# Tariq-Abuhashim/semantic-slam

Measured on AMD Instinct MI355X. Metric: Mvoxels/sec integrated, 512³ grid @ 640×480 depth; achieved HBM GB/s %peak, higher is better.
Workload: dtype f32

## Files before the change

include/tsdf_hip_diag.h:

```cpp
#ifndef TSDF_HIP_DIAG_H
#define TSDF_HIP_DIAG_H

#include "tsdf_hip.h"

#ifdef __cplusplus
extern "C" {
#endif


int tsdf_integrate_sequence_timed(tsdf_volume *vol, const float *depth_dev, const float *cam2world,
                                  int32_t n_frames, float *elapsed_ms);

int tsdf_integrate_frames_timed(tsdf_volume *vol, const float *const *depth_dev, const uint8_t *const *masks_dev,
                                const float *cam2world, int32_t n_frames, float *elapsed_ms);


int tsdf_probe_graph_replay(tsdf_volume *vol, const float *depth_dev, const float *cam2world, int32_t n_frames,
                            int32_t iters, float *ms_launches, float *ms_graph);

int tsdf_probe_stream(tsdf_volume *vol, int32_t non_temporal, int32_t n_iters, float *elapsed_ms);


int tsdf_selftest_fastdiv(int32_t device, uint64_t seed, uint64_t n_samples, float fx, float cx,
                          uint64_t *mismatches, float first_bad[4]);

int tsdf_selftest_fastdiv_band(int32_t device, uint64_t seed, uint64_t n_samples, uint64_t *mismatches,
                               float first_bad[4]);

int tsdf_selftest_round(int32_t device, uint64_t *mismatches, float first_bad[4]);

int tsdf_selftest_tile_tables(int32_t device, const float *depth_dev, const uint8_t *mask_dev, int32_t im_height,
                              int32_t im_width, float max_depth, uint64_t *mismatches);


int32_t tsdf_frames_per_launch(const tsdf_volume *vol);
int tsdf_shortcut_stats(tsdf_volume *vol, int32_t enable, uint64_t counts_out[3]);
int tsdf_brick_list_stats(tsdf_volume *vol, uint64_t counts_out[4]);
int tsdf_classification_info(tsdf_volume *vol, double info_out[2]);

int tsdf_summary_stats(tsdf_volume *vol, uint64_t out[3]);
int tsdf_summary_words(tsdf_volume *vol, uint32_t *out_host, int64_t capacity, int64_t *count);

int tsdf_store_stats(tsdf_volume *vol, int64_t out[9]);

int tsdf_last_cam2base(const tsdf_volume *vol, float out[16]);


int tsdf_set_kernel_variant(tsdf_volume *vol, int32_t variant);

int tsdf_set_brick_shape(tsdf_volume *vol, int32_t quads, int32_t rows, int32_t slices);
int tsdf_brick_shape(const tsdf_volume *vol, int32_t shape_out[3]);
int tsdf_default_brick_shape(const tsdf_config *cfg, int32_t shape_out[3]);

#ifdef __cplusplus
}
#endif
#endif
```

semantic_slam_amd/capi.py:

```python
import ctypes as C
import os

import numpy as np

_PKG = os.path.dirname(os.path.abspath(__file__))
LIB_PATH = os.environ.get("TSDF_HIP_LIB") or os.path.join(_PKG, "libtsdf_hip.so")

ABI_SYMBOLS = [
    "tsdf_config_default", "tsdf_create", "tsdf_destroy", "tsdf_reset", "tsdf_integrate",
    "tsdf_integrate_u16", "tsdf_convert_depth_u16", "tsdf_set_deferral",
    "tsdf_integrate_device", "tsdf_integrate_cam2base", "tsdf_integrate_masked_device",
    "tsdf_integrate_frames_device",
    "tsdf_sync", "tsdf_download", "tsdf_copy_slices", "tsdf_upload", "tsdf_refresh_summary", "tsdf_device_ptrs", "tsdf_slab_voxels", "tsdf_frames_per_launch", "tsdf_shortcut_stats", "tsdf_brick_list_stats", "tsdf_classification_info", "tsdf_store_stats", "tsdf_summary_stats", "tsdf_summary_words",
    "tsdf_get_config", "tsdf_last_cam2base", "tsdf_set_stream", "tsdf_get_stream",
    "tsdf_count_surface", "tsdf_extract_surface", "tsdf_extract_crossings", "tsdf_extract_mesh", "tsdf_save_mesh_ply", "tsdf_save_mesh_welded_ply", "tsdf_save_ply", "tsdf_save_bin", "tsdf_load_bin", "tsdf_save_state", "tsdf_load_state",
    "tsdf_integrate_sequence_timed", "tsdf_integrate_frames_timed", "tsdf_probe_graph_replay", "tsdf_probe_stream", "tsdf_selftest_fastdiv", "tsdf_selftest_fastdiv_band", "tsdf_selftest_round", "tsdf_selftest_tile_tables", "tsdf_set_kernel_variant", "tsdf_set_brick_shape", "tsdf_brick_shape", "tsdf_default_brick_shape", "tsdf_last_error",
    "tsdf_version", "tsdf_multiply_matrix", "tsdf_invert_matrix",
    "tsdf_labels_enable", "tsdf_compose_labels", "tsdf_integrate_labels_device", "tsdf_integrate_frames_labels_device",
    "tsdf_download_labels",
    "tsdf_colour_enable", "tsdf_integrate_colour_device", "tsdf_integrate_rgbd", "tsdf_download_colour",
    "tsdf_raycast_params_default", "tsdf_raycast_device", "tsdf_raycast", "tsdf_batch_raycast_device",
    "tsdf_track_params_default", "tsdf_track", "tsdf_track_system",
    "tsdf_batch_track", "tsdf_batch_track_system", "tsdf_track_member_systems",
    "tsdf_fuse_params_default", "tsdf_fuse_volume",
    "tsdf_align_params_default", "tsdf_fuse_pose_default", "tsdf_align_volume", "tsdf_align_system", "tsdf_fuse_volume_at",
    "tsdf_extent_params_default", "tsdf_volume_extent", "tsdf_batch_extents", "tsdf_group_extent", "tsdf_extent_combine",
    "tsdf_extent_metric", "tsdf_extent_regrid",
    "tsdf_associate_params_default", "tsdf_associate_count", "tsdf_associate_assign", "tsdf_batch_associate",
    "tsdf_segment_params_default", "tsdf_segmenter_create", "tsdf_segmenter_destroy", "tsdf_segmenter_set_stream",
    "tsdf_segment_depth_device", "tsdf_segment_refine_masks_device", "tsdf_segment_frame",
    "tsdf_object_origin", "tsdf_batch_create", "tsdf_batch_destroy", "tsdf_batch_size", "tsdf_batch_volume",
    "tsdf_batch_integrate_device", "tsdf_batch_sync",
    "tsdf_group_create", "tsdf_group_destroy", "tsdf_group_size", "tsdf_group_voxels", "tsdf_group_volume",
    "tsdf_group_integrate", "tsdf_group_integrate_frames", "tsdf_group_set_deferral", "tsdf_group_sync", "tsdf_group_reset", "tsdf_group_download",
    "tsdf_group_extract_surface", "tsdf_group_extract_crossings", "tsdf_group_extract_mesh",
    "tsdf_group_save_ply", "tsdf_group_save_mesh_ply", "tsdf_group_save_bin",
]
DIAG_SYMBOLS = [
    "tsdf_integrate_sequence_timed", "tsdf_integrate_frames_timed",
    "tsdf_probe_graph_replay", "tsdf_probe_stream",
    "tsdf_selftest_fastdiv", "tsdf_selftest_fastdiv_band", "tsdf_selftest_round", "tsdf_selftest_tile_tables",
    "tsdf_shortcut_stats", "tsdf_brick_list_stats", "tsdf_classification_info", "tsdf_store_stats", "tsdf_summary_stats", "tsdf_summary_words", "tsdf_frames_per_launch", "tsdf_last_cam2base",
    "tsdf_set_kernel_variant", "tsdf_set_brick_shape", "tsdf_brick_shape", "tsdf_default_brick_shape",
]


class TsdfError(RuntimeError):
    pass


SHIPPED_VARIANTS = (0, 1, 3, 7, 8)


def experiments_build():
    return b"+experiments" in load().tsdf_version()


def variants(*wanted):
    exp = experiments_build()
    return [v for v in wanted if v in SHIPPED_VARIANTS or exp]


class TsdfConfig(C.Structure):
    _fields_ = [
        ("im_height", C.c_int32), ("im_width", C.c_int32),
# ... 116 lines not shown
    L.tsdf_destroy.argtypes = [vp]
    L.tsdf_reset.argtypes = [vp]
    L.tsdf_integrate.argtypes = [vp, vp, vp]
    L.tsdf_set_deferral.argtypes = [vp, C.c_int32]
    L.tsdf_integrate_u16.argtypes = [vp, vp, C.c_float, C.c_int32, C.c_int32, vp]
    L.tsdf_convert_depth_u16.argtypes = [vp, vp, vp, C.c_float, C.c_int32, C.c_int32]
    L.tsdf_integrate_device.argtypes = [vp, vp, vp]
    L.tsdf_integrate_cam2base.argtypes = [vp, vp, vp]
    L.tsdf_integrate_masked_device.argtypes = [vp, vp, vp, vp]
    L.tsdf_integrate_frames_device.argtypes = [vp, vp, vp, vp, C.c_int32]
    L.tsdf_sync.argtypes = [vp]
    L.tsdf_download.argtypes = [vp, vp, vp]
    L.tsdf_upload.argtypes = [vp, vp, vp]
    L.tsdf_copy_slices.argtypes = [vp, C.c_int32, C.c_int32, vp, vp]
    L.tsdf_refresh_summary.argtypes = [vp]
    L.tsdf_device_ptrs.argtypes = [vp, C.POINTER(vp), C.POINTER(vp)]
    L.tsdf_slab_voxels.argtypes = [vp]
    L.tsdf_slab_voxels.restype = C.c_int64
    L.tsdf_frames_per_launch.argtypes = [vp]
    L.tsdf_frames_per_launch.restype = C.c_int32
    L.tsdf_shortcut_stats.argtypes = [vp, C.c_int32, vp]
    L.tsdf_classification_info.argtypes = [vp, vp]
    L.tsdf_brick_list_stats.argtypes = [vp, vp]
    if hasattr(L, "tsdf_store_stats"):
        L.tsdf_store_stats.argtypes = [vp, i64p]
    if hasattr(L, "tsdf_summary_stats"):
        L.tsdf_summary_stats.argtypes = [vp, vp]
    if hasattr(L, "tsdf_summary_words"):
        L.tsdf_summary_words.argtypes = [vp, vp, C.c_int64, i64p]
    L.tsdf_get_config.argtypes = [vp, C.POINTER(TsdfConfig)]
    L.tsdf_last_cam2base.argtypes = [vp, vp]
    L.tsdf_set_stream.argtypes = [vp, vp]
    L.tsdf_get_stream.argtypes = [vp, C.POINTER(vp)]
    L.tsdf_count_surface.argtypes = [vp, C.c_float, i64p]
    L.tsdf_extract_surface.argtypes = [vp, C.c_float, vp, C.c_int64, i64p]
    L.tsdf_extract_crossings.argtypes = [vp, vp, vp, C.c_float, vp, C.c_int64, i64p]
    L.tsdf_extract_mesh.argtypes = [vp, vp, vp, C.c_float, vp, C.c_int64, i64p]
    L.tsdf_save_mesh_ply.argtypes = [vp, C.c_char_p, C.c_float]
    L.tsdf_save_mesh_welded_ply.argtypes = [vp, C.c_char_p, C.c_float]
    L.tsdf_save_ply.argtypes = [vp, C.c_char_p, C.c_float]
    L.tsdf_save_bin.argtypes = [vp, C.c_char_p]
    L.tsdf_load_bin.argtypes = [vp, C.c_char_p]
    L.tsdf_save_state.argtypes = [vp, C.c_char_p]
    L.tsdf_load_state.argtypes = [vp, C.c_char_p]
    L.tsdf_integrate_sequence_timed.argtypes = [vp, vp, vp, C.c_int32, f32p]
    L.tsdf_integrate_frames_timed.argtypes = [vp, vp, vp, vp, C.c_int32, f32p]
# ... 133 lines not shown


def invert_matrix(m):
    out = np.zeros(16, np.float32)
    m = _f32(m, 16)
    ok = load().tsdf_invert_matrix(m.ctypes.data, out.ctypes.data)
    return bool(ok), out


def selftest_fastdiv(n_samples, seed=1, device=0, fx=535.4, cx=320.1):
    cnt = C.c_uint64()
    bad = (C.c_float * 4)()
    check(load().tsdf_selftest_fastdiv(device, seed, n_samples, fx, cx, C.byref(cnt), bad), "tsdf_selftest_fastdiv")
    return cnt.value, list(bad)


def selftest_fastdiv_band(n_samples, seed=1, device=0):
    cnt = C.c_uint64()
    bad = (C.c_float * 4)()
    check(load().tsdf_selftest_fastdiv_band(device, seed, n_samples, C.byref(cnt), bad), "tsdf_selftest_fastdiv_band")
    return cnt.value, list(bad)


def object_origin(depth_ptr, mask_ptr, h, w, K, device=0):
    k = _f32(K, 9)
    out = np.empty(3, np.float32)
    check(load().tsdf_object_origin(device, depth_ptr, mask_ptr, h, w, k.ctypes.data, out.ctypes.data), "tsdf_object_origin")
    return out


def raycast_params_default(cfg):
    p = RaycastParams()
    check(load().tsdf_raycast_params_default(C.byref(cfg), C.byref(p)), "tsdf_raycast_params_default")
    return p


def track_params_default(cfg):
    p = TrackParams()
    check(load().tsdf_track_params_default(C.byref(cfg), C.byref(p)), "tsdf_track_params_default")
    return p


def fuse_params_default(cfg):
    p = FuseParams()
    check(load().tsdf_fuse_params_default(C.byref(cfg), C.byref(p)), "tsdf_fuse_params_default")
    return p
# ... 184 lines not shown
        return self

    def __exit__(self, *exc):
        self.close()

    def __del__(self):
        try:
            self.close()
        except Exception:
            pass

    @property
    def n_voxels(self):
        return int(self.lib.tsdf_slab_voxels(self._h))

    def shortcut_stats(self, enable=True):
        out = (C.c_uint64 * 3)()
        check(self.lib.tsdf_shortcut_stats(self._h, 1 if enable else 0, out), "tsdf_shortcut_stats")
        return tuple(int(x) for x in out)

    def brick_list_stats(self):
        out = (C.c_uint64 * 4)()
        check(self.lib.tsdf_brick_list_stats(self._h, out), "tsdf_brick_list_stats")
        return tuple(int(x) for x in out)

    def classification_info(self):
        out = (C.c_double * 2)()
        check(self.lib.tsdf_classification_info(self._h, out), "tsdf_classification_info")
        return float(out[0]), int(out[1])

    def store_stats(self):
        out = (C.c_int64 * 9)()
        check(self.lib.tsdf_store_stats(self._h, out), "tsdf_store_stats")
        return {name: tuple(int(x) for x in out[3 * k:3 * k + 3]) for k, name in enumerate(("frames", "masks", "tables"))}

    def summary_stats(self):
        out = (C.c_uint64 * 3)()
        check(self.lib.tsdf_summary_stats(self._h, out), "tsdf_summary_stats")
        return tuple(int(x) for x in out)

    def summary_words(self):
        n = C.c_int64(0)
        check(self.lib.tsdf_summary_words(self._h, None, 0, C.byref(n)), "tsdf_summary_words")
        out = np.zeros(int(n.value), np.uint32)
        if out.size:
            check(self.lib.tsdf_summary_words(self._h, out.ctypes.data, out.size, C.byref(n)), "tsdf_summary_words")
# ... 540 lines not shown
```

semantic_slam_amd/csrc/host_derive.h:

```cpp
#pragma once
#include <algorithm>
#include <cmath>
#include <cstddef>
#include <cstdint>

#include "tsdf_hip.h"

namespace tsdf_host {

inline bool brick_shape_ok(const tsdf_config &c, int q, int r, int s)
{
    return c.dim_x % 4 == 0 && q >= 1 && r >= 1 && s >= 1 && q * r * s <= 64 && (c.dim_x / 4) % q == 0 &&
           (long long)s * c.dim_x * c.dim_y < (1ll << 30);
}

inline void choose_brick_default(const tsdf_config &c, int &bq, int &br, int &bs)
{
    bq = 0; br = 0; bs = 1;
    if (c.dim_x % 4 != 0) return;
    const int quads = c.dim_x / 4;
    const int nz = c.z_end - c.z_begin;
    double best = 1e300;
    for (int q = 1; q <= 64 && q <= quads; ++q) {
        if (quads % q) continue;
// ... 176 lines not shown
constexpr uint32_t kSummaryOnes = 1u, kSummarySane = 2u, kSummaryRun = 4u;
constexpr int kRunCountShift = 8;
constexpr uint32_t kMaxRunCount = (1u << 24) - 1;
constexpr uint32_t kSummaryFresh = kSummaryOnes | kSummarySane | kSummaryRun;

TSDF_HOST_DEVICE inline bool word_has_run(uint32_t word) { return (word & kSummaryRun) != 0u; }
TSDF_HOST_DEVICE inline uint32_t word_run_count(uint32_t word) { return word >> kRunCountShift; }
TSDF_HOST_DEVICE inline uint32_t word_with_run(uint32_t low, uint32_t c)
{
    return (low & (kSummaryOnes | kSummarySane)) | kSummaryRun | (c << kRunCountShift);
}
TSDF_HOST_DEVICE inline uint32_t word_without_run(uint32_t word) { return word & (kSummaryOnes | kSummarySane); }

TSDF_HOST_DEVICE inline uint32_t word_after_update(uint32_t word, bool touched, bool all_updated, bool left_not_one)
{
    if (!touched) return word;
    if (left_not_one) word &= ~kSummaryOnes;
    if (!word_has_run(word)) return word;
    const uint32_t c = word_run_count(word);
    if (!all_updated || c >= kMaxRunCount) return word_without_run(word);
    return word_with_run(word, c + 1u);
}

struct Regions {
    size_t add(size_t bytes) { const size_t at = (end_ + 255) / 256 * 256; end_ = at + bytes; return at; }
    size_t total() const { return end_; }
    size_t end_ = 0;
};

}
```

semantic_slam_amd/csrc/tsdf_diag.hip.h:

```cpp
#pragma once

namespace {

template <typename Queue>
int time_on_stream(tsdf_volume *v, const char *who, float *elapsed_ms, Queue &&queue)
{
    Event e0, e1;
    HIP_TRY(event_create(e0, hipEventDefault));
    HIP_TRY(event_create(e1, hipEventDefault));
    HIP_TRY(hipEventRecord(e0, v->stream));
    const int rc = queue();
    hipError_t er = hipEventRecord(e1, v->stream);
    hipError_t es = hipEventSynchronize(e1);
    float ms = 0.f;
    hipError_t et = hipEventElapsedTime(&ms, e0, e1);
    if (rc) return rc;
    if (er != hipSuccess || es != hipSuccess || et != hipSuccess)
        return fail(TSDF_ERR_HIP, "%s: event timing failed", who);
    *elapsed_ms = ms;
    return TSDF_OK;
}

int frames_timed(tsdf_volume *v, const float *const *depth_dev, const uint8_t *const *masks_dev,
                 const float *cam2world, int32_t n_frames, float *elapsed_ms, const char *who)
// ... 108 lines not shown
    if (e == hipSuccess) e = hipMemcpy(first_bad, d_bad, 4 * sizeof(float), hipMemcpyDeviceToHost);
    if (e != hipSuccess) return fail(TSDF_ERR_HIP, "tsdf_selftest_fastdiv: %s", hipGetErrorString(e));
    *mismatches = cnt;
    return TSDF_OK;
}

int tsdf_selftest_fastdiv_band(int32_t device, uint64_t seed, uint64_t n_samples, uint64_t *mismatches, float first_bad[4])
{
    if (!mismatches || !first_bad) return fail(TSDF_ERR_INVALID, "tsdf_selftest_fastdiv_band: NULL argument");
    HIP_TRY(hipSetDevice(device));
    DevPtr<unsigned long long> d_cnt;
    DevPtr<float> d_bad;
    HIP_TRY(dev_alloc(d_cnt, sizeof(unsigned long long)));
    HIP_TRY(dev_alloc(d_bad, 4 * sizeof(float)));
    HIP_TRY(hipMemset(d_cnt, 0, sizeof(unsigned long long)));
    HIP_TRY(hipMemset(d_bad, 0, 4 * sizeof(float)));
    hipLaunchKernelGGL(tsdfk::selftest_fastdiv_band, dim3(256 * 8), dim3(256), 0, 0, seed, n_samples, d_cnt, d_bad);
    hipError_t e = hipGetLastError();
    if (e == hipSuccess) e = hipDeviceSynchronize();
    unsigned long long cnt = 0;
    if (e == hipSuccess) e = hipMemcpy(&cnt, d_cnt, sizeof cnt, hipMemcpyDeviceToHost);
    if (e == hipSuccess) e = hipMemcpy(first_bad, d_bad, 4 * sizeof(float), hipMemcpyDeviceToHost);
    if (e != hipSuccess) return fail(TSDF_ERR_HIP, "tsdf_selftest_fastdiv_band: %s", hipGetErrorString(e));
    *mismatches = cnt;
    return TSDF_OK;
}

int tsdf_selftest_round(int32_t device, uint64_t *mismatches, float first_bad[4])
{
    if (!mismatches || !first_bad) return fail(TSDF_ERR_INVALID, "tsdf_selftest_round: NULL argument");
    HIP_TRY(hipSetDevice(device));
    DevPtr<unsigned long long> d_cnt;
    DevPtr<float> d_bad;
    HIP_TRY(dev_alloc(d_cnt, sizeof(unsigned long long)));
    HIP_TRY(dev_alloc(d_bad, 4 * sizeof(float)));
    HIP_TRY(hipMemset(d_cnt, 0, sizeof(unsigned long long)));
    HIP_TRY(hipMemset(d_bad, 0, 4 * sizeof(float)));
    hipLaunchKernelGGL(tsdfk::selftest_round, dim3(256 * 8), dim3(256), 0, 0, d_cnt, d_bad);
    hipError_t e = hipGetLastError();
    if (e == hipSuccess) e = hipDeviceSynchronize();
    unsigned long long cnt = 0;
    if (e == hipSuccess) e = hipMemcpy(&cnt, d_cnt, sizeof cnt, hipMemcpyDeviceToHost);
    if (e == hipSuccess) e = hipMemcpy(first_bad, d_bad, 4 * sizeof(float), hipMemcpyDeviceToHost);
    if (e != hipSuccess) return fail(TSDF_ERR_HIP, "tsdf_selftest_round: %s", hipGetErrorString(e));
    *mismatches = cnt;
    return TSDF_OK;
// ... 90 lines not shown
    }
    *mismatches = bad;
    return TSDF_OK;
}


int32_t tsdf_frames_per_launch(const tsdf_volume *v)
{
    if (!v) return 0;
    return can_fuse(v) ? frames_per_launch(v) : 1;
}

int tsdf_shortcut_stats(tsdf_volume *v, int32_t enable, uint64_t counts_out[3])
{
    if (!v) return fail(TSDF_ERR_INVALID, "tsdf_shortcut_stats: NULL handle");
    int rc = bind_device(v);
    if (rc) return rc;
    HIP_TRY(hipStreamSynchronize(v->stream));
    if (counts_out) {
        unsigned int h[3] = {0, 0, 0};
        if (v->d_shortcut_stats) HIP_TRY(hipMemcpy(h, v->d_shortcut_stats, sizeof h, hipMemcpyDeviceToHost));
        for (int i = 0; i < 3; ++i) counts_out[i] = h[i];
    }
    if (enable && !v->d_shortcut_stats) HIP_TRY(dev_alloc(v->d_shortcut_stats, 8 * sizeof(unsigned int)));
    if (v->d_shortcut_stats) {
        if (enable) HIP_TRY(hipMemset(v->d_shortcut_stats, 0, 8 * sizeof(unsigned int)));
        else v->d_shortcut_stats.reset();
    }
    return TSDF_OK;
}

int tsdf_brick_list_stats(tsdf_volume *v, uint64_t counts_out[4])
{
    if (!v || !counts_out) return fail(TSDF_ERR_INVALID, "tsdf_brick_list_stats: NULL argument");
    int rc = bind_device(v);
    if (rc) return rc;
    HIP_TRY(hipStreamSynchronize(v->stream));
    unsigned int h[8] = {0, 0, 0, 0, 0, 0, 0, 0};
    if (v->d_shortcut_stats) HIP_TRY(hipMemcpy(h, v->d_shortcut_stats, sizeof h, hipMemcpyDeviceToHost));
    for (int i = 0; i < 4; ++i) counts_out[i] = h[3 + i];
    return TSDF_OK;
}

int tsdf_classification_info(tsdf_volume *v, double info_out[2])
{
    if (!v || !info_out) return fail(TSDF_ERR_INVALID, "tsdf_classification_info: NULL argument");
    int rc = bind_device(v);
    if (rc) return rc;
    HIP_TRY(hipStreamSynchronize(v->stream));
    if (v->rb_stream) HIP_TRY(hipStreamSynchronize(v->rb_stream));
    if (v->claims_pending && hipEventQuery(v->claims_done) == hipSuccess) {
        v->claim_fraction = claims_read_back(v);
        v->claims_pending = false;
        v->claims_known = true;
    }
    info_out[0] = v->claims_known ? v->claim_fraction : -1.0;
    info_out[1] = (double)v->launches_unclassified;
    return TSDF_OK;
}

int tsdf_summary_stats(tsdf_volume *v, uint64_t out[3])
{
    if (!v || !out) return fail(TSDF_ERR_INVALID, "tsdf_summary_stats: NULL argument");
// ... 85 lines not shown
```

semantic_slam_amd/csrc/tsdf_kernels.hip.h:

```cpp
#pragma once
#include <hip/hip_runtime.h>
#include <stdint.h>
#include <type_traits>

#include "host_derive.h"

namespace tsdfk {

struct IntegrateParams {
    const float *depth;
    const uint8_t *mask;
    float *tsdf;
    float *weight;
    float fx, fy, cx, cy;
    float rx0, rx1, rx2;
    float ry0, ry1, ry2;
    float rz0, rz1, rz2;
    float tx, ty, tz;
    float ox, oy, oz;
    float vs, trunc, max_depth;
    int dim_x, dim_y;
    int nz, z_begin;
    int H, W;
    int xgroups;
    uint32_t *flags;
    int nseg;
    int quads_per_row, quads_per_slice, chunks_per_slice;
    int brick_q, brick_r, brick_s, bricks_per_group, brick_groups;
    int brick_q_magic, brick_per_magic;
    int fast_ok;
// ... 450 lines not shown
        const uint32_t mode = h2 & 7u;
        uint32_t dm = h0 & 0x7fffffu;
        if (mode == 1) dm = 0x7fffffu; else if (mode == 2) dm = 0u; else if (mode == 3) dm &= 0x7u;
        const uint32_t de = 127u - 20u + (h0 >> 23) % 41u;
        const float d = __uint_as_float((de << 23) | dm);
        uint32_t ne = 127u - 81u + (h1 >> 23) % 142u;
        if (mode >= 6) ne = de - 2u + (h1 >> 23) % 5u;
        if (ne > 127u + 60u) ne = 127u + 60u;
        uint32_t nm = h1 & 0x7fffffu;
        if (mode == 4) nm = 0x7fffffu; else if (mode == 5) nm = dm;
        if (ne == 127u + 60u) nm = 0u;
        float n = __uint_as_float((((h2 >> 3) & 1u) << 31) | (ne << 23) | nm);
        if (((h2 >> 5) & 63u) == 0u) n = 0.0f;
        if (((h2 >> 5) & 63u) == 1u) n = __uint_as_float(0x7fc00000u | (h2 >> 12));
        const float q = fast_div_r(n, d, refined_rcp(d));
        const float r = n / d;
        const bool same = __float_as_uint(q) == __float_as_uint(r) || (q != q && r != r);
        if (!same) {
            if (atomicAdd(mismatch, 1ull) == 0ull) { first_bad[0] = n; first_bad[1] = d; first_bad[2] = q; first_bad[3] = r; }
        }
    }
}

__global__ __launch_bounds__(256) void selftest_round(unsigned long long *mismatch, float *first_bad)
{
    const uint64_t stride = (uint64_t)gridDim.x * blockDim.x;
    const uint64_t n_pos = 0x4B800001ull, n_neg = 0x3F000000ull;
    for (uint64_t i = (uint64_t)blockIdx.x * blockDim.x + threadIdx.x; i < n_pos + n_neg; i += stride) {
        const uint32_t bits = i < n_pos ? (uint32_t)i : (0x80000000u + (uint32_t)(i - n_pos));
        const float u = __uint_as_float(bits);
        if (!(u > -0.5f)) continue;
        const int want = (int)roundf(u);
        const int got = round_half_up_i32(u);
        if (got != want) {
            if (atomicAdd(mismatch, 1ull) == 0ull) { first_bad[0] = u; first_bad[1] = (float)got; first_bad[2] = (float)want; first_bad[3] = 0.f; }
        }
    }
}

template <bool NT>
__global__ __launch_bounds__(256) void stream_rmw(float *tsdf, float *weight, size_t n_quads, float one,
                                                  float zero)
{
    const size_t stride = (size_t)gridDim.x * blockDim.x;
    for (size_t q = (size_t)blockIdx.x * blockDim.x + threadIdx.x; q < n_quads; q += stride) {
        float4 t = vol_load<NT>(tsdf + 4 * q);
// ... 112 lines not shown
```

semantic_slam_amd/csrc/tsdf_multiframe.hip.h:

```cpp
#pragma once
#include "launch_geometry.h"
#include "tsdf_kernels.hip.h"

namespace tsdfk {

constexpr int kMaxFramesPerLaunch = 32;
constexpr int kFineTile = 4;
constexpr int kFineLevels = 3;
__host__ __device__ inline size_t fine_table_elems(int fw, int fh) { return (size_t)kFineLevels * kFineLevels * fw * fh; }

struct FramePose {
    const float *depth;
    const uint8_t *mask;
    float rx0, ry0, rx1, ry1, rx2, ry2, rz0, rz1, rz2, tz, tx, ty;
    int fast_ok;
    float cz_margin;
    const uint16_t *label_im;
    const float *score_im;
    const float2 *tiles;
    float cz_short;
    float cz_pad;
};

constexpr int kListBuckets = 64;
// ... 517 lines not shown
    cls[id] = (uint8_t)c;
}

struct LabelState {
    uint16_t *label;
    float *fp, *bp;
    float prob_thd;
};

struct MultiParamsInline {
    IntegrateParams common;
    FramePose frames[kMaxFramesPerLaunch];
    int n_frames;
    LabelState labels;
    int z_fastest;
#ifdef TSDF_EXPERIMENTS
    const unsigned int *super_mask;
    int nz_super;
#endif
};

constexpr int kSuperZ = 4;

template <int R, bool NT, bool FLAT, bool LABELS = false, bool MASKS = true, bool SHORT = false, bool BRICK = false, bool EAGER_W = false>
__device__ __forceinline__ void multi_body(const IntegrateParams &p, const FramePose *__restrict__ frames,
                                           const int n_frames, const int b0, const int b1, const int lz,
                                           const LabelState ls = LabelState(), const unsigned int free_frames = 0u,
                                           const unsigned int skip_frames = 0u)
{
    static_assert(!SHORT || R == 1, "patch classification is written for one row per lane");
    static_assert(!LABELS || R == 1, "label fusion rides on the one-row kernel");
    static_assert(!FLAT || R == 1, "the flat mapping handles one quad per lane");
    static_assert(!BRICK || (R == 1 && !FLAT), "bricks are their own mapping");
    static_assert(!EAGER_W || BRICK, "eager weights are for the bricks of a work list");
    int xg, gy0;
    size_t row0, flag0;
    size_t brick_base = 0;
    unsigned int lane_byte = 0u;
    uint32_t flag32 = 0u;
    constexpr bool kBuf = BRICK && !NT;
    __amdgpu_buffer_rsrc_t t_buf, w_buf;
    auto load_quad = [&](const bool tsdf, const int r) -> float4 {
        if constexpr (kBuf) {
            const v4u v = __builtin_amdgcn_raw_buffer_load_b128(tsdf ? t_buf : w_buf, (int)lane_byte, 0, 0);
            return make_float4(__uint_as_float(v.x), __uint_as_float(v.y), __uint_as_float(v.z), __uint_as_float(v.w));
        } else {
            return vol_load<NT>((tsdf ? p.tsdf : p.weight) + row0 + (size_t)r * p.dim_x);
        }
    };
    auto store_quad = [&](const bool tsdf, const int r, const float4 q) {
        if constexpr (kBuf) {
            const v4u v = {__float_as_uint(q.x), __float_as_uint(q.y), __float_as_uint(q.z), __float_as_uint(q.w)};
            __builtin_amdgcn_raw_buffer_store_b128(v, tsdf ? t_buf : w_buf, (int)lane_byte, 0, 0);
        } else {
            vol_store<NT>((tsdf ? p.tsdf : p.weight) + row0 + (size_t)r * p.dim_x, q);
        }
    };
// ... 49 lines not shown
        t4[r] = make_float4(1.f, 1.f, 1.f, 1.f);
        w4[r] = make_float4(0.f, 0.f, 0.f, 0.f);
        touched[r] = tchanged[r] = false;
    }
    bool have_w = false;
    if constexpr (EAGER_W) {
        w4[0] = load_quad(false, 0);
        have_w = true;
    }

    float bxv[4], byv[R];
#pragma unroll
    for (int j = 0; j < 4; ++j) bxv[j] = p.ox + (float)(xg * 4 + j) * p.vs;
#pragma unroll
    for (int r = 0; r < R; ++r) byv[r] = p.oy + (float)(gy0 + r) * p.vs;
    const float bz = p.oz + (float)gz * p.vs;
    const v2f F = {p.fx, p.fy}, C = {p.cx, p.cy};
    const float trunc_r1 = refined_rcp(p.trunc);
    bool fast_frame = false;

    float diff[R][4];
    bool upd[R][4], rowany[R], bandr[R];
    bool any = false, band = false;
    auto apply_frame = [&]() __attribute__((always_inline)) {
#pragma unroll
        for (int r = 0; r < R; ++r) {
            if (rowany[r] && !touched[r]) {
                if (!have_w) w4[r] = load_quad(false, r);
                if (!(fl[r] & 1u)) t4[r] = load_quad(true, r);
                touched[r] = true;
            }
        }
        float dist[R][4];
        if (__ballot(band) != 0ull) {
            if (fast_frame && p.trunc_fast != 0) {
#pragma unroll
                for (int r = 0; r < R; ++r)
#pragma unroll
                    for (int j = 0; j < 4; ++j) dist[r][j] = fminf(1.0f, fast_div_r(diff[r][j], p.trunc, trunc_r1));
            } else {
#pragma unroll
                for (int r = 0; r < R; ++r)
#pragma unroll
                    for (int j = 0; j < 4; ++j) dist[r][j] = fminf(1.0f, diff[r][j] / p.trunc);
            }
        } else {
#pragma unroll
            for (int r = 0; r < R; ++r)
#pragma unroll
                for (int j = 0; j < 4; ++j) dist[r][j] = 1.0f;
        }

#pragma unroll
        for (int r = 0; r < R; ++r) {
            if (__ballot(!(ones[r] && (fl[r] & 2u)) || bandr[r]) == 0ull) {
                if (upd[r][0]) w4[r].x += 1.0f;
                if (upd[r][1]) w4[r].y += 1.0f;
                if (upd[r][2]) w4[r].z += 1.0f;
                if (upd[r][3]) w4[r].w += 1.0f;
                continue;
            }
            float tv[4] = {t4[r].x, t4[r].y, t4[r].z, t4[r].w};
            float wv[4] = {w4[r].x, w4[r].y, w4[r].z, w4[r].w};
            float num[4], wn[4];
            const bool wave_band = __ballot(bandr[r]) != 0ull;
            bool need = false;
#pragma unroll
            for (int j = 0; j < 4; ++j) {
                wn[j] = wv[j] + 1.0f;
                num[j] = tv[j] * wv[j] + dist[r][j];
            }
            if (!wave_band) {
#pragma unroll
// ... 163 lines not shown
                for (int r = 0; r < R; ++r)
#pragma unroll
                    for (int j = 0; j < 4; ++j) dval[r][j] = dval[r][j] * (mval[r][j] >= 128 ? 1.0f : 0.0f);
            }
        }

#pragma unroll
        for (int r = 0; r < R; ++r) {
            rowany[r] = false;
            bandr[r] = false;
#pragma unroll
            for (int j = 0; j < 4; ++j) {
                const float d = dval[r][j];
                const float df = d - pcz[r][j];
                diff[r][j] = df;
                const bool u = !((d <= 0.0f) | (d > p.max_depth)) & !(df <= -p.trunc);
                upd[r][j] = u;
                rowany[r] |= u;
                bandr[r] |= u & !(df >= p.trunc);
            }
            band |= bandr[r];
            any |= rowany[r];
        }
        if (__ballot(any) == 0ull) continue;

        if constexpr (LABELS) {
            if (q.label_im != nullptr && __ballot(band) != 0ull) {
                uint16_t lab_in[4];
                float sc_in[4];
                bool hit = false;
#pragma unroll
                for (int j = 0; j < 4; ++j) {
                    const bool seen = upd[0][j] & (diff[0][j] < p.trunc);
                    lab_in[j] = 0;
                    sc_in[j] = 0.0f;
                    if (seen) { lab_in[j] = q.label_im[pixel[0][j]]; sc_in[j] = q.score_im[pixel[0][j]]; }
                    hit |= lab_in[j] != 0;
                }
                if (hit) {
                    ushort4 L4 = *reinterpret_cast<const ushort4 *>(ls.label + row0);
                    float4 F4 = *reinterpret_cast<const float4 *>(ls.fp + row0);
                    float4 B4 = *reinterpret_cast<const float4 *>(ls.bp + row0);
                    uint16_t L[4] = {L4.x, L4.y, L4.z, L4.w};
                    float Fv[4] = {F4.x, F4.y, F4.z, F4.w}, Bv[4] = {B4.x, B4.y, B4.z, B4.w};
#pragma unroll
                    for (int j = 0; j < 4; ++j) {
                        const uint16_t l = lab_in[j];
                        const float sc = sc_in[j];
                        if (l == 0) continue;
                        if (L[j] == 0) { L[j] = l; Fv[j] = sc; Bv[j] = 0.0f; }
                        else if (L[j] == l) { Fv[j] = Fv[j] + sc; }
                        else {
                            Bv[j] = Bv[j] + sc;
                            if (Fv[j] / (Fv[j] + Bv[j]) < ls.prob_thd) { L[j] = l; Fv[j] = sc; Bv[j] = 0.0f; }
                        }
                    }
                    ushort4 Lo; Lo.x = L[0]; Lo.y = L[1]; Lo.z = L[2]; Lo.w = L[3];
                    *reinterpret_cast<ushort4 *>(ls.label + row0) = Lo;
                    *reinterpret_cast<float4 *>(ls.fp + row0) = make_float4(Fv[0], Fv[1], Fv[2], Fv[3]);
                    *reinterpret_cast<float4 *>(ls.bp + row0) = make_float4(Bv[0], Bv[1], Bv[2], Bv[3]);
                }
            }
        }

        }

        apply_frame();
    }

#pragma unroll
    for (int r = 0; r < R; ++r) {
        const bool store_t = __ballot(touched[r] && tchanged[r]) != 0ull;
        if (touched[r]) {
            if (store_t) store_quad(true, r, t4[r]);
            store_quad(false, r, w4[r]);
        }
        if ((fl[r] & 1u) && !ones[r]) {
            if constexpr (BRICK) {
                p.flags[flag32] = fl[r] & 2u;
            } else {
                p.flags[flag0 + (size_t)r * p.nseg] = fl[r] & 2u;
            }
        }
    }
}

#ifndef TSDF_BRICK_WAVES
#define TSDF_BRICK_WAVES 8
#endif
template <int R, bool NT, bool FLAT, bool LABELS = false, bool MASKS = true>
__global__ __launch_bounds__(256, R == 2 ? 6 : 1) void integrate_multi_inline(MultiParamsInline mp)
{
    typedef const char __attribute__((address_space(4))) *kernarg_ptr;
    kernarg_ptr base = (kernarg_ptr)__builtin_amdgcn_kernarg_segment_ptr();
    typedef const FramePose __attribute__((address_space(4))) *frames_ptr;
    frames_ptr frames = (frames_ptr)(base + offsetof(MultiParamsInline, frames));
    const int wg_x = mp.z_fastest ? (int)blockIdx.z : (int)blockIdx.x, wg_y = (int)blockIdx.y;
    int wg_z = mp.z_fastest ? (int)blockIdx.x : (int)blockIdx.z;
    if (mp.z_fastest == 2) {
        wg_z += (int)((unsigned)(wg_x + wg_y) % gridDim.x);
        if (wg_z >= (int)gridDim.x) wg_z -= (int)gridDim.x;
    }
    multi_body<R, NT, FLAT, LABELS, MASKS>(mp.common, (const FramePose *)frames, mp.n_frames, wg_x, wg_y, wg_z, mp.labels);
}

constexpr int kSuperBX = 4, kSuperBY = 2, kSuperBZ = 1;
constexpr int kSuperBricks = kSuperBX * kSuperBY * kSuperBZ;
static_assert(kSuperBricks <= 32, "one lane of a half-wave per brick of the super-brick");
constexpr unsigned int kBrickUndecided = 0x80000000u;

struct BrickListParams {
    uint4 *list;
    unsigned char *counters;
    unsigned int bucket_cap;
    ClassPoseTable *poses;
    int nsx, nsy, nsz;
    int wedge_mode, wedge_oy, wedge_oz, super_h, super_d, fy_px;
};


__global__ __launch_bounds__(256) void classify_brick_list(MultiParamsInline mp, BrickListParams bl)
{
    typedef const char __attribute__((address_space(4))) *kernarg_ptr;
    kernarg_ptr base = (kernarg_ptr)__builtin_amdgcn_kernarg_segment_ptr();
    const FramePose *frames = (const FramePose *)(base + offsetof(MultiParamsInline, frames));
    const IntegrateParams &p = mp.common;
// ... 76 lines not shown
        const int lane = threadIdx.x;
        const unsigned int frames_mask = mp.n_frames >= 32 ? 0xffffffffu : ((1u << mp.n_frames) - 1u);
        const int g = brick / p.bricks_per_group, i = brick - g * p.bricks_per_group;
        const int xa = i * p.brick_q * 4, ya = g * p.brick_r;
        const int z0 = zg * p.brick_s, z1 = min(z0 + p.brick_s - 1, p.nz - 1);
        const float2 *fine_f = p.fine != nullptr ? p.fine + (size_t)(lane & 31) * fine_table_elems(p.fine_w, p.fine_h) : nullptr;
        const int cls = classify_patch<true>(p, class_pose(poses, lane & 31), xa, xa + p.brick_q * 4 - 1, ya, min(ya + p.brick_r - 1, p.dim_y - 1),
                                             p.z_begin + z0, p.z_begin + z1, fine_f);
        free_frames |= (unsigned int)__ballot(cls == 1) & frames_mask;
        skip_frames |= (unsigned int)__ballot(cls == 2) & frames_mask;
        free_frames = __builtin_amdgcn_readfirstlane(free_frames);
        skip_frames = __builtin_amdgcn_readfirstlane(skip_frames);
        if (skip_frames == frames_mask) {
            if (p.shortcut_stats != nullptr && lane == 0) { atomicAdd(p.shortcut_stats + 2, (unsigned)mp.n_frames); atomicAdd(p.shortcut_stats + 6, 1u); }
            return;
        }
    }
    multi_body<1, NT, false, LABELS, MASKS, true, true, true>(mp.common, frames, mp.n_frames, brick, 0, zg, mp.labels, free_frames, skip_frames);
}

template <bool NT, bool FLAT>
__global__ __launch_bounds__(256) void integrate_multi_single(IntegrateParams p, FramePose pose)
{
    multi_body<1, NT, FLAT>(p, &pose, 1, blockIdx.x, blockIdx.y, blockIdx.z);
}

template <bool NT>
__global__ __launch_bounds__(256) void integrate_multi_batched(const IntegrateParams *__restrict__ params,
                                                               const FramePose *__restrict__ poses,
                                                               const int2 *__restrict__ slice_map)
{
    const int2 m = slice_map[blockIdx.z];
    const IntegrateParams p = params[m.x];
    multi_body<1, NT, true>(p, poses + m.x, 1, blockIdx.x, 0, m.y);
}

template <bool NT>
__global__ __launch_bounds__(256, 8) void integrate_single_bricks(IntegrateParams p, FramePose pose)
{
    const unsigned c = p.wg_class[(blockIdx.x + gridDim.x * blockIdx.z) * 4u + threadIdx.y];
    if (c == 2u) return;
    multi_body<1, NT, false, false, true, true, true>(p, &pose, 1, (int)blockIdx.x * 4 + __builtin_amdgcn_readfirstlane((int)threadIdx.y), 0,
                                                      blockIdx.z, LabelState(), c == 1u ? 1u : 0u, 0u);
}

template <bool NT>
__global__ __launch_bounds__(256, 8) void integrate_multi_batched_bricks(const IntegrateParams *__restrict__ params,
// ... 34 lines not shown
```

Before: 493,100.

## Add dense-frame fast path tracking uniform weight count per wave

```diff
diff --git a/include/tsdf_hip_diag.h b/include/tsdf_hip_diag.h
--- a/include/tsdf_hip_diag.h
+++ b/include/tsdf_hip_diag.h
@@ -27,6 +27,9 @@
 int tsdf_selftest_fastdiv_band(int32_t device, uint64_t seed, uint64_t n_samples, uint64_t *mismatches,
                                float first_bad[4]);
 
+int tsdf_selftest_fastdiv_count(int32_t device, uint64_t seed, uint32_t per_divisor, uint64_t *mismatches,
+                                float first_bad[4]);
+
 int tsdf_selftest_round(int32_t device, uint64_t *mismatches, float first_bad[4]);
 
 int tsdf_selftest_tile_tables(int32_t device, const float *depth_dev, const uint8_t *mask_dev, int32_t im_height,
@@ -36,6 +39,7 @@
 int32_t tsdf_frames_per_launch(const tsdf_volume *vol);
 int tsdf_shortcut_stats(tsdf_volume *vol, int32_t enable, uint64_t counts_out[3]);
 int tsdf_brick_list_stats(tsdf_volume *vol, uint64_t counts_out[4]);
+int tsdf_dense_frame_stats(tsdf_volume *vol, uint64_t counts_out[2]);
 int tsdf_classification_info(tsdf_volume *vol, double info_out[2]);
 
 int tsdf_summary_stats(tsdf_volume *vol, uint64_t out[3]);
diff --git a/semantic_slam_amd/capi.py b/semantic_slam_amd/capi.py
--- a/semantic_slam_amd/capi.py
+++ b/semantic_slam_amd/capi.py
@@ -11,10 +11,10 @@
     "tsdf_integrate_u16", "tsdf_convert_depth_u16", "tsdf_set_deferral",
     "tsdf_integrate_device", "tsdf_integrate_cam2base", "tsdf_integrate_masked_device",
     "tsdf_integrate_frames_device",
-    "tsdf_sync", "tsdf_download", "tsdf_copy_slices", "tsdf_upload", "tsdf_refresh_summary", "tsdf_device_ptrs", "tsdf_slab_voxels", "tsdf_frames_per_launch", "tsdf_shortcut_stats", "tsdf_brick_list_stats", "tsdf_classification_info", "tsdf_store_stats", "tsdf_summary_stats", "tsdf_summary_words",
+    "tsdf_sync", "tsdf_download", "tsdf_copy_slices", "tsdf_upload", "tsdf_refresh_summary", "tsdf_device_ptrs", "tsdf_slab_voxels", "tsdf_frames_per_launch", "tsdf_shortcut_stats", "tsdf_brick_list_stats", "tsdf_dense_frame_stats", "tsdf_classification_info", "tsdf_store_stats", "tsdf_summary_stats", "tsdf_summary_words",
     "tsdf_get_config", "tsdf_last_cam2base", "tsdf_set_stream", "tsdf_get_stream",
     "tsdf_count_surface", "tsdf_extract_surface", "tsdf_extract_crossings", "tsdf_extract_mesh", "tsdf_save_mesh_ply", "tsdf_save_mesh_welded_ply", "tsdf_save_ply", "tsdf_save_bin", "tsdf_load_bin", "tsdf_save_state", "tsdf_load_state",
-    "tsdf_integrate_sequence_timed", "tsdf_integrate_frames_timed", "tsdf_probe_graph_replay", "tsdf_probe_stream", "tsdf_selftest_fastdiv", "tsdf_selftest_fastdiv_band", "tsdf_selftest_round", "tsdf_selftest_tile_tables", "tsdf_set_kernel_variant", "tsdf_set_brick_shape", "tsdf_brick_shape", "tsdf_default_brick_shape", "tsdf_last_error",
+    "tsdf_integrate_sequence_timed", "tsdf_integrate_frames_timed", "tsdf_probe_graph_replay", "tsdf_probe_stream", "tsdf_selftest_fastdiv", "tsdf_selftest_fastdiv_band", "tsdf_selftest_fastdiv_count", "tsdf_selftest_round", "tsdf_selftest_tile_tables", "tsdf_set_kernel_variant", "tsdf_set_brick_shape", "tsdf_brick_shape", "tsdf_default_brick_shape", "tsdf_last_error",
     "tsdf_version", "tsdf_multiply_matrix", "tsdf_invert_matrix",
     "tsdf_labels_enable", "tsdf_compose_labels", "tsdf_integrate_labels_device", "tsdf_integrate_frames_labels_device",
     "tsdf_download_labels",
@@ -39,8 +39,8 @@
 DIAG_SYMBOLS = [
     "tsdf_integrate_sequence_timed", "tsdf_integrate_frames_timed",
     "tsdf_probe_graph_replay", "tsdf_probe_stream",
-    "tsdf_selftest_fastdiv", "tsdf_selftest_fastdiv_band", "tsdf_selftest_round", "tsdf_selftest_tile_tables",
-    "tsdf_shortcut_stats", "tsdf_brick_list_stats", "tsdf_classification_info", "tsdf_store_stats", "tsdf_summary_stats", "tsdf_summary_words", "tsdf_frames_per_launch", "tsdf_last_cam2base",
+    "tsdf_selftest_fastdiv", "tsdf_selftest_fastdiv_band", "tsdf_selftest_fastdiv_count", "tsdf_selftest_round", "tsdf_selftest_tile_tables",
+    "tsdf_shortcut_stats", "tsdf_brick_list_stats", "tsdf_dense_frame_stats", "tsdf_classification_info", "tsdf_store_stats", "tsdf_summary_stats", "tsdf_summary_words", "tsdf_frames_per_launch", "tsdf_last_cam2base",
     "tsdf_set_kernel_variant", "tsdf_set_brick_shape", "tsdf_brick_shape", "tsdf_default_brick_shape",
 ]
 
@@ -203,6 +203,9 @@
     L.tsdf_shortcut_stats.argtypes = [vp, C.c_int32, vp]
     L.tsdf_classification_info.argtypes = [vp, vp]
     L.tsdf_brick_list_stats.argtypes = [vp, vp]
+    if hasattr(L, "tsdf_dense_frame_stats"):
+        L.tsdf_dense_frame_stats.argtypes = [vp, vp]
+        L.tsdf_selftest_fastdiv_count.argtypes = [C.c_int32, C.c_uint64, C.c_uint32, C.POINTER(C.c_uint64), f32p]
     if hasattr(L, "tsdf_store_stats"):
         L.tsdf_store_stats.argtypes = [vp, i64p]
     if hasattr(L, "tsdf_summary_stats"):
@@ -382,6 +385,13 @@
     return cnt.value, list(bad)
 
 
+def selftest_fastdiv_count(per_divisor, seed=1, device=0):
+    cnt = C.c_uint64()
+    bad = (C.c_float * 4)()
+    check(load().tsdf_selftest_fastdiv_count(device, seed, per_divisor, C.byref(cnt), bad), "tsdf_selftest_fastdiv_count")
+    return cnt.value, list(bad)
+
+
 def object_origin(depth_ptr, mask_ptr, h, w, K, device=0):
     k = _f32(K, 9)
     out = np.empty(3, np.float32)
@@ -612,6 +622,11 @@
     def brick_list_stats(self):
         out = (C.c_uint64 * 4)()
         check(self.lib.tsdf_brick_list_stats(self._h, out), "tsdf_brick_list_stats")
+        return tuple(int(x) for x in out)
+
+    def dense_frame_stats(self):
+        out = (C.c_uint64 * 2)()
+        check(self.lib.tsdf_dense_frame_stats(self._h, out), "tsdf_dense_frame_stats")
         return tuple(int(x) for x in out)
 
     def classification_info(self):
diff --git a/semantic_slam_amd/csrc/host_derive.h b/semantic_slam_amd/csrc/host_derive.h
--- a/semantic_slam_amd/csrc/host_derive.h
+++ b/semantic_slam_amd/csrc/host_derive.h
@@ -222,6 +222,35 @@
     return word_with_run(word, c + 1u);
 }
 
+TSDF_HOST_DEVICE inline bool dense_count_ok(float c) { return c >= 0.0f && c <= 16777215.0f && c == (float)(int32_t)c; }
+
+constexpr float kDenseCountMax = 16777215.0f;
+struct DenseRun {
+    bool alive = true;
+    bool started = false;
+    float c = 0.0f;
+};
+
+TSDF_HOST_DEVICE inline bool dense_frame(DenseRun &s, bool full, bool uniform, float w)
+{
+    if (!s.alive) return false;
+    if (!full) { s.alive = false; return false; }
+    if (!s.started) {
+        if (!uniform || !dense_count_ok(w)) { s.alive = false; return false; }
+        s.started = true;
+        s.c = w;
+    } else if (!(s.c <= kDenseCountMax)) {
+        s.alive = false;
+        return false;
+    }
+    return true;
+}
+
+TSDF_HOST_DEVICE inline void dense_advance(DenseRun &s) { s.c = s.c + 1.0f; }
+
+constexpr float kDenseNumMin = 8.673617379884035e-19f;
+constexpr float kDenseNumEnd = 33554432.0f;
+
 struct Regions {
     size_t add(size_t bytes) { const size_t at = (end_ + 255) / 256 * 256; end_ = at + bytes; return at; }
     size_t total() const { return end_; }
diff --git a/semantic_slam_amd/csrc/tsdf_diag.hip.h b/semantic_slam_amd/csrc/tsdf_diag.hip.h
--- a/semantic_slam_amd/csrc/tsdf_diag.hip.h
+++ b/semantic_slam_amd/csrc/tsdf_diag.hip.h
@@ -154,6 +154,27 @@
     if (e == hipSuccess) e = hipMemcpy(&cnt, d_cnt, sizeof cnt, hipMemcpyDeviceToHost);
     if (e == hipSuccess) e = hipMemcpy(first_bad, d_bad, 4 * sizeof(float), hipMemcpyDeviceToHost);
     if (e != hipSuccess) return fail(TSDF_ERR_HIP, "tsdf_selftest_fastdiv_band: %s", hipGetErrorString(e));
+    *mismatches = cnt;
+    return TSDF_OK;
+}
+
+int tsdf_selftest_fastdiv_count(int32_t device, uint64_t seed, uint32_t per_divisor, uint64_t *mismatches, float first_bad[4])
+{
+    if (!mismatches || !first_bad || per_divisor == 0u) return fail(TSDF_ERR_INVALID, "tsdf_selftest_fastdiv_count: NULL argument or no numerators");
+    HIP_TRY(hipSetDevice(device));
+    DevPtr<unsigned long long> d_cnt;
+    DevPtr<float> d_bad;
+    HIP_TRY(dev_alloc(d_cnt, sizeof(unsigned long long)));
+    HIP_TRY(dev_alloc(d_bad, 4 * sizeof(float)));
+    HIP_TRY(hipMemset(d_cnt, 0, sizeof(unsigned long long)));
+    HIP_TRY(hipMemset(d_bad, 0, 4 * sizeof(float)));
+    hipLaunchKernelGGL(tsdfk::selftest_fastdiv_count, dim3(256 * 8), dim3(256), 0, 0, seed, per_divisor, d_cnt, d_bad);
+    hipError_t e = hipGetLastError();
+    if (e == hipSuccess) e = hipDeviceSynchronize();
+    unsigned long long cnt = 0;
+    if (e == hipSuccess) e = hipMemcpy(&cnt, d_cnt, sizeof cnt, hipMemcpyDeviceToHost);
+    if (e == hipSuccess) e = hipMemcpy(first_bad, d_bad, 4 * sizeof(float), hipMemcpyDeviceToHost);
+    if (e != hipSuccess) return fail(TSDF_ERR_HIP, "tsdf_selftest_fastdiv_count: %s", hipGetErrorString(e));
     *mismatches = cnt;
     return TSDF_OK;
 }
@@ -290,9 +311,9 @@
         if (v->d_shortcut_stats) HIP_TRY(hipMemcpy(h, v->d_shortcut_stats, sizeof h, hipMemcpyDeviceToHost));
         for (int i = 0; i < 3; ++i) counts_out[i] = h[i];
     }
-    if (enable && !v->d_shortcut_stats) HIP_TRY(dev_alloc(v->d_shortcut_stats, 8 * sizeof(unsigned int)));
+    if (enable && !v->d_shortcut_stats) HIP_TRY(dev_alloc(v->d_shortcut_stats, tsdfk::kShortcutStatWords * sizeof(unsigned int)));
     if (v->d_shortcut_stats) {
-        if (enable) HIP_TRY(hipMemset(v->d_shortcut_stats, 0, 8 * sizeof(unsigned int)));
+        if (enable) HIP_TRY(hipMemset(v->d_shortcut_stats, 0, tsdfk::kShortcutStatWords * sizeof(unsigned int)));
         else v->d_shortcut_stats.reset();
     }
     return TSDF_OK;
@@ -307,6 +328,18 @@
     unsigned int h[8] = {0, 0, 0, 0, 0, 0, 0, 0};
     if (v->d_shortcut_stats) HIP_TRY(hipMemcpy(h, v->d_shortcut_stats, sizeof h, hipMemcpyDeviceToHost));
     for (int i = 0; i < 4; ++i) counts_out[i] = h[3 + i];
+    return TSDF_OK;
+}
+
+int tsdf_dense_frame_stats(tsdf_volume *v, uint64_t counts_out[2])
+{
+    if (!v || !counts_out) return fail(TSDF_ERR_INVALID, "tsdf_dense_frame_stats: NULL argument");
+    int rc = bind_device(v);
+    if (rc) return rc;
+    HIP_TRY(hipStreamSynchronize(v->stream));
+    unsigned int h[tsdfk::kShortcutStatWords] = {};
+    if (v->d_shortcut_stats) HIP_TRY(hipMemcpy(h, v->d_shortcut_stats, sizeof h, hipMemcpyDeviceToHost));
+    for (int i = 0; i < 2; ++i) counts_out[i] = h[7 + i];
     return TSDF_OK;
 }
 
diff --git a/semantic_slam_amd/csrc/tsdf_kernels.hip.h b/semantic_slam_amd/csrc/tsdf_kernels.hip.h
--- a/semantic_slam_amd/csrc/tsdf_kernels.hip.h
+++ b/semantic_slam_amd/csrc/tsdf_kernels.hip.h
@@ -6,6 +6,8 @@
 #include "host_derive.h"
 
 namespace tsdfk {
+
+constexpr int kShortcutStatWords = 9;
 
 struct IntegrateParams {
     const float *depth;
@@ -502,6 +504,43 @@
     }
 }
 
+__global__ __launch_bounds__(256) void selftest_fastdiv_count(uint64_t seed, uint32_t per_divisor, unsigned long long *mismatch,
+                                                              float *first_bad)
+{
+    const uint32_t stride = gridDim.x * blockDim.x;
+    const uint32_t lo_bits = (127u - 60u) << 23, end_bits = (127u + 25u) << 23;
+    for (uint32_t di = blockIdx.x * blockDim.x + threadIdx.x + 1u; di <= (1u << 24); di += stride)
+    for (uint32_t k = 0; k < per_divisor; ++k) {
+        const uint64_t i = (uint64_t)(di - 1u) * per_divisor + k;
+        const float d = (float)di;
+        const uint32_t h0 = hash32(seed + 2 * i), h1 = hash32(seed + 2 * i + 1);
+        const uint32_t mode = k & 15u;
+        const uint32_t ne = 127u - 60u + (h0 >> 23) % 85u;
+        uint32_t nb;
+        if (mode == 0u) nb = (ne << 23) | 0x7fffffu;
+        else if (mode == 1u) nb = ne << 23;
+        else if (mode == 2u) nb = (ne << 23) | (__float_as_uint(d) & 0x7fffffu);
+        else if (mode == 3u) nb = (ne << 23) | (h1 & 7u);
+        else if (mode <= 5u) nb = lo_bits + (h1 & 0xffu);
+        else if (mode <= 7u) nb = end_bits - 1u - (h1 & 0xffu);
+        else if (mode <= 11u) {
+            const uint32_t most = (1u << 25) / di;
+            const uint32_t m = 1u + h1 % most;
+            nb = __float_as_uint((float)m * d);
+            if (mode == 10u) nb += 1u;
+            if (mode == 11u) nb -= 1u;
+        } else nb = (ne << 23) | (h1 & 0x7fffffu);
+        if (nb >= end_bits) nb = end_bits - 1u;
+        if (nb < lo_bits) nb = lo_bits;
+        const float n = __uint_as_float(nb | ((h0 & 1u) << 31));
+        const float q = fast_div_r(n, d, refined_rcp(d));
+        const float r = n / d;
+        if (__float_as_uint(q) != __float_as_uint(r)) {
+            if (atomicAdd(mismatch, 1ull) == 0ull) { first_bad[0] = n; first_bad[1] = d; first_bad[2] = q; first_bad[3] = r; }
+        }
+    }
+}
+
 __global__ __launch_bounds__(256) void selftest_round(unsigned long long *mismatch, float *first_bad)
 {
     const uint64_t stride = (uint64_t)gridDim.x * blockDim.x;
diff --git a/semantic_slam_amd/csrc/tsdf_multiframe.hip.h b/semantic_slam_amd/csrc/tsdf_multiframe.hip.h
--- a/semantic_slam_amd/csrc/tsdf_multiframe.hip.h
+++ b/semantic_slam_amd/csrc/tsdf_multiframe.hip.h
@@ -563,7 +563,8 @@
 
 constexpr int kSuperZ = 4;
 
-template <int R, bool NT, bool FLAT, bool LABELS = false, bool MASKS = true, bool SHORT = false, bool BRICK = false, bool EAGER_W = false>
+template <int R, bool NT, bool FLAT, bool LABELS = false, bool MASKS = true, bool SHORT = false, bool BRICK = false, bool EAGER_W = false,
+          bool DENSE = false>
 __device__ __forceinline__ void multi_body(const IntegrateParams &p, const FramePose *__restrict__ frames,
                                            const int n_frames, const int b0, const int b1, const int lz,
                                            const LabelState ls = LabelState(), const unsigned int free_frames = 0u,
@@ -574,6 +575,7 @@
     static_assert(!FLAT || R == 1, "the flat mapping handles one quad per lane");
     static_assert(!BRICK || (R == 1 && !FLAT), "bricks are their own mapping");
     static_assert(!EAGER_W || BRICK, "eager weights are for the bricks of a work list");
+    static_assert(!DENSE || (R == 1 && !BRICK && !LABELS && !SHORT), "dense frames are written for the per-voxel one-row kernels");
     int xg, gy0;
     size_t row0, flag0;
     size_t brick_base = 0;
@@ -669,6 +671,7 @@
     float diff[R][4];
     bool upd[R][4], rowany[R], bandr[R];
     bool any = false, band = false;
+    tsdf_host::DenseRun dense;
     auto apply_frame = [&]() __attribute__((always_inline)) {
 #pragma unroll
         for (int r = 0; r < R; ++r) {
@@ -696,6 +699,58 @@
             for (int r = 0; r < R; ++r)
 #pragma unroll
                 for (int j = 0; j < 4; ++j) dist[r][j] = 1.0f;
+        }
+
+        if constexpr (DENSE) {
+            bool run_dense = false;
+            if (dense.alive) {
+                const bool counting = dense.started;
+                const bool full = __ballot(bandr[0]) != 0ull &&
+                                  __popcll(__ballot(upd[0][0] && upd[0][1] && upd[0][2] && upd[0][3])) == 64;
+                bool uniform = false;
+                float w = 0.0f;
+                if (full && !counting) {
+                    const uint32_t wb = (uint32_t)__builtin_amdgcn_readfirstlane((int)__float_as_uint(w4[0].x));
+                    const bool same = __float_as_uint(w4[0].x) == wb && __float_as_uint(w4[0].y) == wb &&
+                                      __float_as_uint(w4[0].z) == wb && __float_as_uint(w4[0].w) == wb;
+                    uniform = __ballot(!same) == 0ull;
+                    w = __uint_as_float(wb);
+                }
+                run_dense = tsdf_host::dense_frame(dense, full, uniform, w);
+                if (counting && !dense.alive) w4[0] = make_float4(dense.c, dense.c, dense.c, dense.c);
+            }
+            if (run_dense) {
+                const float c = dense.c, wn = c + 1.0f;
+                const float tv[4] = {t4[0].x, t4[0].y, t4[0].z, t4[0].w};
+                float num[4], nt[4];
+#pragma unroll
+                for (int j = 0; j < 4; ++j) num[j] = tv[j] * c + dist[0][j];
+                bool in = true;
+#pragma unroll
+                for (int j = 0; j < 4; ++j) in &= fabsf(num[j]) < tsdf_host::kDenseNumEnd;
+                in &= fminf(fminf(fabsf(num[0]), fabsf(num[1])), fminf(fabsf(num[2]), fabsf(num[3]))) >= tsdf_host::kDenseNumMin;
+                const bool guarded = __builtin_amdgcn_ballot_w64(!in) == 0ull;
+                if (guarded) {
+                    const float r1 = refined_rcp(wn);
+#pragma unroll
+                    for (int j = 0; j < 4; ++j) nt[j] = fast_div_r(num[j], wn, r1);
+                } else {
+#pragma unroll
+                    for (int j = 0; j < 4; ++j) nt[j] = num[j] / wn;
+                }
+                bool notone = false;
+#pragma unroll
+                for (int j = 0; j < 4; ++j) notone |= __float_as_uint(nt[j]) != 0x3f800000u;
+                t4[0] = make_float4(nt[0], nt[1], nt[2], nt[3]);
+                tchanged[0] = true;
+                if (__builtin_amdgcn_ballot_w64(notone) != 0ull) ones[0] = false;
+                if (p.shortcut_stats != nullptr && (threadIdx.x & 63) == 0) {
+                    atomicAdd(p.shortcut_stats + 7, 1u);
+                    if (!guarded) atomicAdd(p.shortcut_stats + 8, 1u);
+                }
+                tsdf_host::dense_advance(dense);
+                return;
+            }
         }
 
 #pragma unroll
@@ -905,7 +960,13 @@
             band |= bandr[r];
             any |= rowany[r];
         }
-        if (__ballot(any) == 0ull) continue;
+        if (__ballot(any) == 0ull) {
+            if constexpr (DENSE) {
+                if (dense.alive && dense.started) w4[0] = make_float4(dense.c, dense.c, dense.c, dense.c);
+                dense.alive = false;
+            }
+            continue;
+        }
 
         if constexpr (LABELS) {
             if (q.label_im != nullptr && __ballot(band) != 0ull) {
@@ -951,6 +1012,9 @@
         apply_frame();
     }
 
+    if constexpr (DENSE) {
+        if (dense.alive && dense.started) w4[0] = make_float4(dense.c, dense.c, dense.c, dense.c);
+    }
 #pragma unroll
     for (int r = 0; r < R; ++r) {
         const bool store_t = __ballot(touched[r] && tchanged[r]) != 0ull;
@@ -984,7 +1048,8 @@
         wg_z += (int)((unsigned)(wg_x + wg_y) % gridDim.x);
         if (wg_z >= (int)gridDim.x) wg_z -= (int)gridDim.x;
     }
-    multi_body<R, NT, FLAT, LABELS, MASKS>(mp.common, (const FramePose *)frames, mp.n_frames, wg_x, wg_y, wg_z, mp.labels);
+    multi_body<R, NT, FLAT, LABELS, MASKS, false, false, false, R == 1 && !LABELS>(mp.common, (const FramePose *)frames, mp.n_frames, wg_x, wg_y,
+                                                                                    wg_z, mp.labels);
 }
 
 constexpr int kSuperBX = 4, kSuperBY = 2, kSuperBZ = 1;
@@ -1107,7 +1172,7 @@
 template <bool NT, bool FLAT>
 __global__ __launch_bounds__(256) void integrate_multi_single(IntegrateParams p, FramePose pose)
 {
-    multi_body<1, NT, FLAT>(p, &pose, 1, blockIdx.x, blockIdx.y, blockIdx.z);
+    multi_body<1, NT, FLAT, false, true, false, false, false, true>(p, &pose, 1, blockIdx.x, blockIdx.y, blockIdx.z);
 }
 
 template <bool NT>
```

Result: no change. 494,000 (median of 3 runs) (+0.2%).
